# j04n-f/Encrypt-zkVM

Measured on AMD Instinct MI355X. Metric: STARK prove: trace-steps/sec at 2^20 steps; achieved HBM GB/s vs 8 TB/s peak, higher is better.
Workload: dtype f128

## Files before the change

encrypt-zkvm_amd/csrc/f128.hpp:

```cpp
#pragma once
#include <hip/hip_runtime.h>
#include <stdint.h>

#include "addsub_asm.hpp"

#define ZK_HD __host__ __device__ __forceinline__

struct fe {
    uint64_t lo, hi;
};

static constexpr uint64_t ZK_P_LO = 0xffffd30000000001ULL;
static constexpr uint64_t ZK_P_HI = 0xffffffffffffffffULL;
static constexpr uint64_t ZK_C = 0x2cffffffffffULL;

ZK_HD fe fe_make(uint64_t lo, uint64_t hi = 0) { return fe{lo, hi}; }
ZK_HD fe fe_zero() { return fe{0, 0}; }
ZK_HD fe fe_one() { return fe{1, 0}; }
ZK_HD bool fe_eq(fe a, fe b) { return a.lo == b.lo && a.hi == b.hi; }
ZK_HD bool fe_is_zero(fe a) { return (a.lo | a.hi) == 0; }

ZK_HD uint32_t lo32(uint64_t v) { return (uint32_t)v; }
ZK_HD uint32_t hi32(uint64_t v) { return (uint32_t)(v >> 32); }
ZK_HD uint64_t join32(uint32_t lo, uint32_t hi) { return (uint64_t)lo | ((uint64_t)hi << 32); }
// ... 553 lines not shown
#pragma unroll
    for (int k = 1; k < 8; k++) acc.w[k] = __builtin_addc(acc.w[k], r[k], c, &c);
    acc.w[8] += c;
}
ZK_HD fe acc288_reduce(const acc288 &acc) {
    const fe v = reduce_fold(acc.w[0], acc.w[1], acc.w[2], acc.w[3], acc.w[4], acc.w[5], acc.w[6], acc.w[7]);
    constexpr uint64_t C2_LO = (uint64_t)(((unsigned __int128)ZK_C * ZK_C) & ~0ULL);
    constexpr uint64_t C2_HI = (uint64_t)(((unsigned __int128)ZK_C * ZK_C) >> 64);
    const uint64_t t_lo = (uint64_t)lo32(C2_LO) * acc.w[8];
    const uint64_t t_mid = (uint64_t)hi32(C2_LO) * acc.w[8] + (t_lo >> 32);
    const uint64_t t_hi = C2_HI * acc.w[8] + (t_mid >> 32);
    const fe top = fe{(t_lo & 0xffffffffull) | (t_mid << 32), t_hi};
    return fe_add(v, top);
}

__device__ __forceinline__ fe fe_mul(fe a, fe b) { return fe_mul_asm(a, b); }
__host__ static inline fe fe_from_u128(unsigned __int128 v) { return fe{(uint64_t)v, (uint64_t)(v >> 64)}; }
__host__ static inline unsigned __int128 fe_to_u128(fe a) { return ((unsigned __int128)a.hi << 64) | a.lo; }
__host__ static inline fe fe_reduce_wide(unsigned __int128 lo, unsigned __int128 hi) {
    typedef unsigned __int128 u128;
    const u128 P = ((u128)ZK_P_HI << 64) | ZK_P_LO;
    const u128 t0 = (u128)(uint64_t)hi * ZK_C, t1 = (u128)(uint64_t)(hi >> 64) * ZK_C;
    const u128 s1 = lo + t0;
    const u128 s2 = s1 + (t1 << 64);
    const uint64_t top = (uint64_t)(t1 >> 64) + (uint64_t)(s1 < lo) + (uint64_t)(s2 < s1);
    u128 r = s2 + (u128)top * ZK_C;
    if (r < s2) r += ZK_C;
    if (r >= P) r -= P;
    return fe_from_u128(r);
}
// ... 111 lines not shown
```

encrypt-zkvm_amd/csrc/kernels.hip:

```cpp
#include <hip/hip_runtime.h>
#include <bitset>
#include <mutex>
#include <stdlib.h>
#include <string.h>

#include "blake3.hpp"
#include "fri_small.hpp"
#include "rescue_consts.hpp"
#include "zk_internal.hpp"

namespace zk {

#define ZK_LAUNCH_CHECK() (void)hipGetLastError()

static inline unsigned cdiv(size_t a, size_t b) { return (unsigned)((a + b - 1) / b); }

__device__ __forceinline__ fe ld_fe(const fe *p) { return *p; }
__device__ __forceinline__ void st_fe(fe *p, fe v) { *p = v; }

template <class T>
__device__ __forceinline__ T pow_split(const T *lo, const T *hi, size_t t) {
    return ChalOf<T>::mul(lo[t & 2047], hi[t >> 11]);
}

// ... 1316 lines not shown
                                468778791690ull, 208346129640ull, 22570830711ull, 573956280ull,
                                418414128120ull, 151093990710ull, 15496819560ull, 387420489ull};
    uint32_t pos[6] = {0x0u, 0x200u, 0xffa60000u, 0xffffffffu, 0xffffffffu, 0x1ffu}, neg[6] = {0, 0, 0, 0, 0, 0};
    acc192_madd(pos, y[0], A[4 * r + 0]);
    acc192_madd(neg, y[1], A[4 * r + 1]);
    acc192_madd(pos, y[2], A[4 * r + 2]);
    acc192_madd(neg, y[3], A[4 * r + 3]);
    uint32_t d[6], b;
    d[0] = __builtin_subc(pos[0], neg[0], 0u, &b);
#pragma unroll
    for (int k = 1; k < 6; k++) d[k] = __builtin_subc(pos[k], neg[k], b, &b);
    return reduce_fold(d[0], d[1], d[2], d[3], d[4], d[5], 0u, 0u);
}
static constexpr fe ZK_INV3_72 = fe{0x8092deb1ab776293ull, 0xf0185d00eca40a3bull};

struct EvalShared {
    fe ct[20], cb[22], ct2[20], cb2[22];
    fe ct3[4], nct[4], ct3b[4], nctb[4];
    fe u[4], ub[4];
    fe delta, bnd1, bnd1b;
};

#ifndef ZK_EVAL_LAZY
#define ZK_EVAL_LAZY 1
#endif
#ifndef ZK_EVAL_WAVES
#define ZK_EVAL_WAVES 4
#endif
#ifndef ZK_EVAL_WAVES_EXT
#define ZK_EVAL_WAVES_EXT 4
#endif
template <int KE, bool BND>
__global__ void __launch_bounds__(256, KE == 1 ? ZK_EVAL_WAVES : ZK_EVAL_WAVES_EXT) k_eval_constraints(const fe *lde, int log_n, EvalMap map, const fe *periodic,
                                                          const fe *divs, const AirConsts *K, const AirConsts *K2,
                                                          size_t plane, fe *comp) {
    __shared__ EvalShared S;
    __shared__ fe stash[4][256];
    const int tid = threadIdx.x;
    {
        const int t = threadIdx.x;
        if (t < 20) S.ct[t] = K->coeff_t[t];
        else if (t < 42) S.cb[t - 20] = K->coeff_b[t - 20];
        else if (t == 42) S.bnd1 = K->bnd1;
        else if (t == 43) S.bnd1b = KE == 2 ? K2->bnd1 : fe_zero();
        else if (t == 44) S.delta = K->delta;
        else if (t >= 80 && t < 84) {
            S.ct3[t - 80] = fe_mul(K->coeff_t[12 + t - 80], ZK_INV3_72);
            S.nct[t - 80] = fe_neg(K->coeff_t[12 + t - 80]);
        } else if (KE == 2 && t >= 84 && t < 88) {
            S.ct3b[t - 84] = fe_mul(K2->coeff_t[12 + t - 84], ZK_INV3_72);
            S.nctb[t - 84] = fe_neg(K2->coeff_t[12 + t - 84]);
        }
        else if (t >= 88 && t < 92) S.u[t - 88] = air_fold_mds(K->coeff_t + 12, t - 88);
        else if (KE == 2 && t >= 92 && t < 96) S.ub[t - 92] = air_fold_mds(K2->coeff_t + 12, t - 92);
        else if (KE == 2 && t >= 128 && t < 148) S.ct2[t - 128] = K2->coeff_t[t - 128];
        else if (KE == 2 && t >= 148 && t < 170) S.cb2[t - 148] = K2->coeff_b[t - 148];
        __syncthreads();
    }
    const int L = K->lwe_size;
    const size_t n = (size_t)1 << log_n;
    const size_t CE = n * map.nce;
    const size_t t_id = blockIdx.x * (size_t)blockDim.x + threadIdx.x;
    if (t_id >= CE) return;
    const size_t jl = t_id >> log_n, q = t_id & (n - 1), qn = (q + 1) & (n - 1);
    const size_t rc = map.ce0 + map.cestep * jl;
    const size_t i = rc + 8 * q;
    const size_t r = jl << map.lshift;
    const fe *cb = lde + r * n;
    const size_t cs = (size_t)map.lde_cosets * n;
#define CUR(c) cb[(size_t)(c)*cs + q]
#define NXT(c) cb[(size_t)(c)*cs + qn]
    const fe one = fe_one();
    fe t = fe_zero();
    fe t2 = fe_zero();
#define ZK_ACC(k, val)                                                    \
    do {                                                                  \
        const fe v_ = (val);                                              \
        t = fe_add(t, fe_mul(S.ct[k], v_));                               \
        if (KE == 2) {                                                    \
            t2 = fe_add(t2, fe_mul(S.ct2[k], v_));                        \
            asm volatile("" : "+v"(t2.lo), "+v"(t2.hi));                  \
        }                                                                 \
    } while (0)
    {
        constexpr bool LZ = KE == 1 && ZK_EVAL_LAZY;
        acc288 aS = acc288_zero();
#define ZK_ACCS(k, val)                                  \
    do {                                                 \
        if (LZ) acc288_madd(aS, S.ct[k], (val));    \
        else ZK_ACC(k, val);                             \
    } while (0)
#define ZK_SEQS() ZK_SEQ(cb, LZ ? aS.w[0] : (uint32_t)t.lo)
        const fe b0 = CUR(5), b1 = CUR(4), b2 = CUR(3), b3 = CUR(2), b4 = CUR(1);
        {
            fe opc = b0;
            opc = fe_add(fe_add(opc, opc), b1);
            opc = fe_add(fe_add(opc, opc), b2);
            opc = fe_add(fe_add(opc, opc), b3);
            opc = fe_add(fe_add(opc, opc), b4);
            stash[0][tid] = opc;
        }
        const fe nb0 = fe_sub(one, b0), nb2 = fe_sub(one, b2), nb3 = fe_sub(one, b3), nb4 = fe_sub(one, b4);
        const fe s0 = CUR(12), s1 = CUR(13);
        const fe s0n = NXT(12);
        ZK_ACCS(0, fe_sub(NXT(0), fe_add(CUR(0), one)));
        const fe b01 = fe_mul(b0, b1);
        ZK_ACCS(2, b01);
        const fe b0n1 = fe_sub(b0, b01);
        const fe n0_1 = fe_sub(b1, b01);
        const fe n01 = fe_sub(nb0, n0_1);
        {
            const fe is_noop = fe_mul(fe_mul(fe_mul(n01, nb2), nb3), nb4);
            ZK_ACCS(11, fe_mul(is_noop, fe_sub(s0n, s0)));
        }
        ZK_SEQS();
        const fe n0_1_b2 = fe_mul(n0_1, b2);
        const fe n0_1_n2 = fe_sub(n0_1, n0_1_b2);
        const fe Y = fe_mul(n0_1_n2, b3);
        fe is_add2, is_read2;
        {
            const fe X = fe_sub(n0_1_n2, Y);
            const fe e3 = fe_mul(S.ct[3], fe_sub(s0n, fe_add(s0, s1)));
            const fe e6 = fe_mul(S.ct[6], fe_sub(s0n, fe_mul(s0, s1)));
            const fe i36 = fe_add(e3, fe_mul(b4, fe_sub(e6, e3)));
            if (LZ) acc288_madd(aS, X, i36);
            else t = fe_add(t, fe_mul(X, i36));
            if (KE == 2) {
                const fe f3 = fe_mul(S.ct2[3], fe_sub(s0n, fe_add(s0, s1)));
                const fe f6 = fe_mul(S.ct2[6], fe_sub(s0n, fe_mul(s0, s1)));
                t2 = fe_add(t2, fe_mul(X, fe_add(f3, fe_mul(b4, fe_sub(f6, f3)))));
                asm volatile("" : "+v"(t2.lo), "+v"(t2.hi));
            }
        }
        ZK_SEQS();
        {
            is_add2 = fe_mul(Y, b4);
            const fe is_sadd = fe_sub(Y, is_add2);
            const fe is_smul = fe_mul(fe_mul(n0_1_b2, nb3), nb4);
            fe sum_sn = fe_zero(), sum_s1 = fe_zero(), sum_hi = fe_zero();
            for (int k = 0; k < L; k++) {
                sum_sn = fe_add(sum_sn, NXT(12 + k));
                sum_s1 = fe_add(sum_s1, CUR(13 + k));
            }
            for (int k = 1; k < L; k++) sum_hi = fe_add(sum_hi, CUR(12 + L + k));
            const fe base = fe_sub(sum_sn, sum_s1);
            const fe acc7 = fe_sub(sum_sn, fe_mul(sum_s1, s0));
            const fe acc4 = fe_sub(base, fe_mul(S.delta, s0));
            const fe acc5 = fe_sub(base, fe_add(s0, sum_hi));
            ZK_ACCS(4, fe_mul(is_sadd, acc4));
            ZK_ACCS(5, fe_mul(is_add2, acc5));
            ZK_ACCS(7, fe_mul(is_smul, acc7));
        }
        ZK_SEQS();
        {
            const fe p0 = fe_mul(b0n1, nb2);
            const fe p0b3 = fe_mul(p0, b3);
            const fe p0n3 = fe_sub(p0, p0b3);
            stash[1][tid] = fe_mul(s0n, fe_mul(p0n3, nb4));
            is_read2 = fe_mul(p0b3, nb4);
            const fe zd1 = fe_mul(p0n3, fe_sub(NXT(13), s0));
            const fe i89 = fe_add(S.ct[8], fe_mul(b4, fe_sub(S.ct[9], S.ct[8])));
            if (LZ) acc288_madd(aS, zd1, i89);
            else t = fe_add(t, fe_mul(zd1, i89));
            if (KE == 2) {
                t2 = fe_add(t2, fe_mul(zd1, fe_add(S.ct2[8], fe_mul(b4, fe_sub(S.ct2[9], S.ct2[8])))));
                asm volatile("" : "+v"(t2.lo), "+v"(t2.hi));
            }
            ZK_ACCS(10, fe_mul(is_read2, fe_sub(NXT(17), s0)));
        }
        {
            fe v = fe_add(fe_sub(fe_sub(NXT(11), CUR(11)), b0), b1);
            fe d = fe_sub(is_add2, is_read2);
            d = fe_add(d, d);
            d = fe_add(d, d);
            ZK_ACCS(1, fe_add(v, d));
        }
        if (LZ) t = fe_add(t, acc288_reduce(aS));
#undef ZK_ACCS
#undef ZK_SEQS
    }
    ZK_SEQ(cb, t.lo);
    {
        const fe opc = stash[0][tid], push_term = stash[1][tid];
        const fe *per = periodic + (i & 127) * 9;
        acc288 aR = acc288_zero(), aR2 = acc288_zero();
        {
            const fe pv = K->pv[i & 127];
            aR.w[0] = lo32(pv.lo), aR.w[1] = hi32(pv.lo), aR.w[2] = lo32(pv.hi), aR.w[3] = hi32(pv.hi);
            acc288_madd(aR, S.nct[0], opc);
            acc288_madd(aR, S.nct[1], push_term);
            if (KE == 2) {
                const fe pvb = K2->pv[i & 127];
                aR2.w[0] = lo32(pvb.lo), aR2.w[1] = hi32(pvb.lo), aR2.w[2] = lo32(pvb.hi), aR2.w[3] = hi32(pvb.hi);
                acc288_madd(aR2, S.nctb[0], opc);
                acc288_madd(aR2, S.nctb[1], push_term);
            }
        }
#pragma unroll
        for (int k = 0; k < 4; k++) {
            const fe c = CUR(7 + k);
            if (k < 2) stash[2 + k][tid] = c;
            const fe x = cube(c);
            acc288_madd(aR, S.u[k], x);
            if (KE == 2) acc288_madd(aR2, S.ub[k], x);
        }
        ZK_SEQ(cb, aR.w[0]);
        const fe h0 = CUR(6);
        const fe fh = fe_mul(per[0], h0);
        const fe nfh = fe_sub(h0, fh);
        fe y[4];
#pragma unroll
        for (int k = 0; k < 4; k++) y[k] = fe_sub(NXT(7 + k), per[5 + k]);
        fe sR = fe_zero(), sR2 = fe_zero();
        {
#pragma unroll
            for (int r2 = 0; r2 < 4; r2++) {
                const fe v3 = cube(adj_row(r2, y));
                acc288_madd(aR, S.ct3[r2], v3);
                if (KE == 2) acc288_madd(aR2, S.ct3b[r2], v3);
            }
            sR = acc288_reduce(aR);
            if (KE == 2) sR2 = acc288_reduce(aR2);
        }
        t = fe_add(t, fe_mul(sR, fh));
        if (KE == 2) t2 = fe_add(t2, fe_mul(sR2, fh));
        ZK_SEQ(cb, t.lo);
        {
            const fe c7 = stash[2][tid], c8 = stash[3][tid];
            const fe d16 = fe_sub(NXT(7), c7), d17 = fe_sub(NXT(8), c8), n9 = NXT(9), n10 = NXT(10);
            acc288 aC = acc288_zero();
            acc288_madd(aC, S.ct[16], d16);
            acc288_madd(aC, S.ct[17], d17);
            acc288_madd(aC, S.ct[18], n9);
            acc288_madd(aC, S.ct[19], n10);
            t = fe_add(t, fe_mul(acc288_reduce(aC), nfh));
            if (KE == 2) {
                acc288 aD = acc288_zero();
                acc288_madd(aD, S.ct2[16], d16);
                acc288_madd(aD, S.ct2[17], d17);
                acc288_madd(aD, S.ct2[18], n9);
                acc288_madd(aD, S.ct2[19], n10);
                t2 = fe_add(t2, fe_mul(acc288_reduce(aD), nfh));
            }
        }
    }
    ZK_SEQ(cb, t.lo);
    const size_t P = map.dplane ? map.dplane : CE;
    const fe dT = divs[t_id];
    if constexpr (!BND) {
        comp[t_id] = fe_mul(t, dT);
        if (KE == 2) comp[plane + t_id] = fe_mul(t2, dT);
    } else {
        const fe d0 = divs[P + t_id], d1 = divs[2 * P + t_id];
        acc288 a0 = acc288_zero(), a1 = acc288_zero();
        acc288_madd(a0, S.cb[0], CUR(0));
        acc288_madd(a0, S.cb[1], CUR(7));
        acc288_madd(a0, S.cb[2], CUR(8));
        acc288_madd(a0, S.cb[3], CUR(11));
        acc288_madd(a1, S.cb[12], CUR(7));
        acc288_madd(a1, S.cb[13], CUR(8));
#pragma unroll
        for (int k = 0; k < 8; k++) {
            fe c = CUR(12 + k);
            acc288_madd(a0, S.cb[4 + k], c);
            acc288_madd(a1, S.cb[14 + k], c);
        }
        const fe bs0 = acc288_reduce(a0), bs1 = fe_sub(acc288_reduce(a1), S.bnd1);
        acc288 aR = acc288_zero();
        acc288_madd(aR, t, dT);
        acc288_madd(aR, bs0, d0);
        acc288_madd(aR, bs1, d1);
        const fe res = acc288_reduce(aR);
        comp[t_id] = res;
        if (KE == 2) {
            ZK_SEQ(cb, res.lo);
            acc288 c0 = acc288_zero(), c1 = acc288_zero();
            acc288_madd(c0, S.cb2[0], CUR(0));
            acc288_madd(c0, S.cb2[1], CUR(7));
            acc288_madd(c0, S.cb2[2], CUR(8));
            acc288_madd(c0, S.cb2[3], CUR(11));
            acc288_madd(c1, S.cb2[12], CUR(7));
            acc288_madd(c1, S.cb2[13], CUR(8));
#pragma unroll
            for (int k = 0; k < 8; k++) {
                fe c = CUR(12 + k);
                acc288_madd(c0, S.cb2[4 + k], c);
                acc288_madd(c1, S.cb2[14 + k], c);
            }
            const fe bs0b = acc288_reduce(c0), bs1b = fe_sub(acc288_reduce(c1), S.bnd1b);
            acc288 aR2 = acc288_zero();
            acc288_madd(aR2, t2, dT);
            acc288_madd(aR2, bs0b, d0);
            acc288_madd(aR2, bs1b, d1);
            comp[plane + t_id] = acc288_reduce(aR2);
        }
    }
#undef ZK_ACC
#undef CUR
#undef NXT
}

static std::mutex g_consts_mu;
static std::bitset<256> g_consts_done;
hipError_t upload_rescue_consts(hipStream_t st) {
    int dev = 0;
    hipError_t e = hipGetDevice(&dev);
    if (e != hipSuccess) return e;
    if (dev < 0 || dev >= 256) return hipErrorInvalidDevice;
    std::lock_guard<std::mutex> lk(g_consts_mu);
    if (g_consts_done.test((size_t)dev)) return hipSuccess;
    fe m[16];
// ... 178 lines not shown
            atomicMin(&rep->t_first[tid], mn);
        }
    } else if (tid == 20) {
        atomicAdd(&rep->failing_steps, (unsigned long long)sh_steps[0] + sh_steps[1] + sh_steps[2] + sh_steps[3]);
    }
}

hipError_t validate_trace(hipStream_t st, const fe *trace, size_t n, const fe *per_tab, fe delta, int lwe_size,
                          ValReport *rep) {
    const size_t steps = n - 2;
    ZK_PROF(st, "validate_trace", 448.0 * n, hipLaunchKernelGGL(k_validate_trace, dim3(cdiv(steps, 256)), dim3(256), 0, st,
                                                                trace, n, per_tab, delta, lwe_size, rep));
    return hipGetLastError();
}

__global__ void __launch_bounds__(256) k_comp_cross(CrossMap m, const fe *wi_lo, const fe *wi_hi,
                                                    const fe *i3_lo, const fe *i3_hi, fe scale, fe w8inv,
                                                    fe inv3n, int ncols, fe *polys, unsigned *nonzero) {
    for (size_t kl = blockIdx.x * (size_t)blockDim.x + threadIdx.x; kl < m.kcount; kl += (size_t)gridDim.x * blockDim.x) {
        const size_t k1 = m.k0 + kl;
        fe w = pow_split(wi_lo, wi_hi, k1);
        fe d[8];
        fe wr = fe_one();
#pragma unroll
        for (int r = 0; r < 8; r++) {
            if (r == 7 && m.derive7) {
                acc288 a7 = acc288_zero();
#pragma unroll
                for (int j = 0; j < 7; j++) acc288_madd(a7, m.k7[j], d[j]);
                d[7] = acc288_reduce(a7);
                break;
            }
            fe v = m.c[r][kl];
            d[r] = r ? fe_mul(v, wr) : v;
            wr = fe_mul(wr, w);
        }
        fe w2 = fe_mul(w8inv, w8inv), w3 = fe_mul(w2, w8inv);
        fe e0 = d[0], e1 = d[4], e2 = d[2], e3 = d[6], e4 = d[1], e5 = d[5], e6 = d[3], e7 = d[7];
        fe t0 = fe_add(e0, e1), t1 = fe_sub(e0, e1), t2 = fe_add(e2, e3), t3 = fe_sub(e2, e3);
        fe t4 = fe_add(e4, e5), t5 = fe_sub(e4, e5), t6 = fe_add(e6, e7), t7 = fe_sub(e6, e7);
        t3 = fe_mul(t3, w2);
        t7 = fe_mul(t7, w2);
        fe u0 = fe_add(t0, t2), u2 = fe_sub(t0, t2), u1 = fe_add(t1, t3), u3 = fe_sub(t1, t3);
        fe u4 = fe_add(t4, t6), u6 = fe_sub(t4, t6), u5 = fe_add(t5, t7), u7 = fe_sub(t5, t7);
        u5 = fe_mul(u5, w8inv);
        u6 = fe_mul(u6, w2);
        u7 = fe_mul(u7, w3);
        fe bk[8] = {fe_add(u0, u4), fe_add(u1, u5), fe_add(u2, u6), fe_add(u3, u7),
                    fe_sub(u0, u4), fe_sub(u1, u5), fe_sub(u2, u6), fe_sub(u3, u7)};
        fe s = fe_mul(scale, pow_split(i3_lo, i3_hi, k1));
        unsigned nz = 0;
#pragma unroll
        for (int k2 = 0; k2 < 8; k2++) {
            fe a = fe_mul(bk[k2], s);
            if (k2 < ncols) polys[(size_t)k2 * m.pstride + kl] = a;
            else nz |= !fe_is_zero(a);
            s = fe_mul(s, inv3n);
        }
        if (nz) atomicOr(nonzero, 1u);
    }
}

void comp_cross_mapped(hipStream_t st, const CrossMap &m, const NttTables &T8n, const PowTable &inv3, fe scale,
                       fe w8inv, fe inv3n, int ncols, fe *polys, unsigned *nonzero_flag) {
    unsigned blocks = cdiv(m.kcount, 256);
    if (blocks > 65536) blocks = 65536;
    ZK_PROF(st, "comp_cross", (128.0 + 16.0 * ncols) * m.kcount, hipLaunchKernelGGL(k_comp_cross, dim3(blocks), dim3(256), 0, st, m, T8n.inv_lo,
                                                 T8n.inv_hi, inv3.lo, inv3.hi, scale, w8inv, inv3n, ncols, polys,
                                                 nonzero_flag));
}

constexpr int OOD_GROUP = 7;

template <int KX>
__global__ void k_ood_tables(typename Chal<KX>::T z, typename Chal<KX>::T zg, uint64_t chunk, int nw,
                             typename Chal<KX>::T *tab) {
    typedef typename Chal<KX>::T T;
    const int t = blockIdx.x * blockDim.x + threadIdx.x;
    if (t >= 128 + 2 * nw) return;
    T x;
    uint64_t e;
    if (t < 128) {
        x = t < 64 ? z : zg;
// ... 663 lines not shown
        if (op == 14) fe_mul_wsv2(x, ws[t], a[mir], ws[mir], o[0], o[1]);
        else fe_mul_w2_2(x, w2[t], a[mir], w2[mir], o[0], o[1]);
        r = o[t & 1];
        break;
    }
    case 16: r = ws_fold(lo32(x.lo), hi32(x.lo), lo32(x.hi), hi32(x.hi), lo32(y.lo), hi32(y.lo) & 7u); break;
    case 17: {
        const fe x2 = a[mir], y2 = b[mir];
        uint32_t A[4] = {lo32(x.lo), hi32(x.lo), lo32(x.hi), hi32(x.hi)};
        uint32_t B[4] = {lo32(x2.lo), hi32(x2.lo), lo32(x2.hi), hi32(x2.hi)};
        fe o[2];
        ws_fold2(A, lo32(y.lo), hi32(y.lo) & 7u, B, lo32(y2.lo), hi32(y2.lo) & 7u, o[0], o[1]);
        r = o[t & 1];
        break;
    }
    case 0: r = fe_add(x, y); break;
    case 1: r = fe_sub(x, y); break;
    case 2: r = fe_mul(x, y); break;
    case 3: r = fe_inv(x); break;
    case 5: r = fe_add_lazy(x, y); break;
    case 6: r = fe_canon(x); break;
    case 7: r = fe_mul_w2(x, fe_w2{y, fe_mul(y, fe{0, 1})}); break;
    case 8:
    case 9:
    case 10: {
        const fe x2 = a[count - 1 - t], y2 = b[count - 1 - t];
        fe o[4];
        if (op == 8) addsub2_v<0>(x, y, x2, y2, o[0], o[1], o[2], o[3]);
        else if (op == 9) addsub2_v<1>(x, y, x2, y2, o[0], o[1], o[2], o[3]);
        else addsub2_v<2>(x, y, x2, y2, o[0], o[1], o[2], o[3]);
// ... 25 lines not shown
```

encrypt-zkvm_amd/csrc/prover.hip:

```cpp
#include <hip/hip_runtime.h>
#include <stdio.h>
#include <string.h>

#include <algorithm>
#include <chrono>
#include <cstdlib>
#include <map>
#include <memory>
#include <new>
#include <string>
#include <vector>

#include "host_pool.hpp"
#include "prover_internal.hpp"
#include "rescue_consts.hpp"

namespace zk {
thread_local std::string g_err;
struct HostTimer {
    bool on = getenv("ZK_HOST_TIMING") != nullptr;
    std::chrono::steady_clock::time_point t = std::chrono::steady_clock::now();
    std::string log;
    void start() { t = std::chrono::steady_clock::now(); }
    void lap(const char *what) { stop(what), start(); }
// ... 734 lines not shown
    e.push_back(fe_make(((uint64_t)opt->field_extension << 16) | ((uint64_t)opt->fri_folding << 8) | opt->fri_rem_max_deg));
    e.push_back(fe_make(opt->grinding));
    e.push_back(fe_make(opt->blowup));
    e.push_back(fe_make(opt->num_queries));
    for (int i = 0; i < 2; i++) e.push_back(fe_from_bytes(pub->program_hash[i]));
    for (int i = 0; i < 16; i++) e.push_back(fe_from_bytes(pub->stack_outputs[i]));
    Coin coin;
    coin.init(e);
    return coin;
}

static void set_coeff_derived(AirConsts &K, const fe *per) {
    K.bnd1 = fe_zero();
    for (int k = 12; k < NUM_ASSERTS; k++) K.bnd1 = fe_add(K.bnd1, fe_mul(K.coeff_b[k], K.assert_val[k]));
    air_fold_periodic(K.coeff_t + 12, per, K.pv);
}

static const fe *air_static_consts(const zk_pub_inputs *pub, size_t n, AirConsts &K) {
    const int log_n = ilog2(n);
    const int first_cols[12] = {0, 7, 8, 11, 12, 13, 14, 15, 16, 17, 18, 19};
    int k = 0;
    for (int i = 0; i < 12; i++, k++) {
        K.assert_col[k] = first_cols[i];
        K.assert_grp[k] = 0;
        K.assert_val[k] = fe_zero();
    }
    for (int i = 0; i < 2; i++, k++) {
        K.assert_col[k] = 7 + i;
        K.assert_grp[k] = 1;
        K.assert_val[k] = fe_from_bytes(pub->program_hash[i]);
// ... 1164 lines not shown
    for (size_t i = 0; i < count; i++) acc288_madd(acc, fe_from_bytes(a + 16 * i), fe_from_bytes(b + 16 * i));
    fe_to_bytes(acc288_reduce(acc), out);
}

extern "C" void zk_diag_mul_limbs_host(const uint8_t *a, const uint8_t *b, uint8_t *out, size_t count) {
    for (size_t i = 0; i < count; i++) fe_to_bytes(fe_mul_limbs(fe_from_bytes(a + 16 * i), fe_from_bytes(b + 16 * i)), out + 16 * i);
}
extern "C" void zk_diag_air_fold_host(const uint8_t *ct, size_t n, uint8_t *u_out, uint8_t *pv_out) {
    fe c[4], pv[128];
    for (int r = 0; r < 4; r++) c[r] = fe_from_bytes(ct + 16 * r);
    for (int k = 0; k < 4; k++) fe_to_bytes(air_fold_mds(c, k), u_out + 16 * k);
    const std::vector<fe> per = periodic_table(n);
    air_fold_periodic(c, per.data(), pv);
    for (int j = 0; j < 128; j++) fe_to_bytes(pv[j], pv_out + 16 * j);
}
extern "C" void zk_diag_blake3_host(const uint8_t *in, size_t len, uint8_t out[32]) { b3::hash_bytes(in, len, out); }

static UploadPlanIn diag_upload_plan_in(const uint32_t *in, size_t n) {
    UploadPlanIn q;
    q.have = in[0], q.sparse = in[1], q.nw8 = in[2], q.nw32 = in[3], q.clk_off = in[4], q.fixed_off = in[5];
    q.snap = in[6], q.snap_mask = in[7], q.hint_ok = in[8], q.no_virtual = in[9], q.lat_sched = in[10], q.detect = in[11];
    q.sparse_on = in[12] & 1u, q.narrow_on = in[12] & 2u, q.clock_on = in[12] & 4u, q.fixed_on = in[12] & 8u;
    q.fixed_fuse_on = in[12] & 16u, q.virtual_on = in[12] & 32u, q.coeff_src_on = in[12] & 64u;
    q.n = n;
    return q;
}
extern "C" int zk_diag_upload_plan_coeff_src(const uint32_t *in, size_t n) {
    return upload_plan(diag_upload_plan_in(in, n)).coeff_src ? 1 : 0;
}
extern "C" int zk_diag_upload_plan(const uint32_t *in, size_t n, uint32_t *masks, int32_t *counts, int32_t *cols,
// ... 39 lines not shown
    if (!idx || !out || (G != 2 && G != 4 && G != 8) || M < 8 * (uint64_t)G || (M & (M - 1)))
        ZK_FAIL(ZK_ERR_INVALID_ARG, "zk_diag_shard_locate: G = 2, 4 or 8, M a power of two >= 8 G");
    TreeGeom T;
    T.shape(M, G);
    for (size_t i = 0; i < count; i++) {
        if (is_node ? (idx[i] < 1 || idx[i] >= M) : idx[i] >= M)
            ZK_FAIL(ZK_ERR_INVALID_ARG, "zk_diag_shard_locate: leaf index below M, heap node index in 1 .. M - 1");
        const TreeGeom::Loc L = T.locate(is_node, idx[i]);
        out[3 * i] = L.owner, out[3 * i + 1] = L.which, out[3 * i + 2] = (int64_t)L.off;
    }
    return ZK_OK;
}

extern "C" int zk_diag_field_op(int device, int op, const uint8_t *a, const uint8_t *b, uint8_t *out, size_t count) {
    if (!a || !b || !out || count == 0) ZK_FAIL(ZK_ERR_INVALID_ARG, "null argument");
    if (op < 0 || op > 17 || count > ((size_t)1 << 30) || (op == 13 && count % 64 != 0))
        ZK_FAIL(ZK_ERR_INVALID_ARG, "zk_diag_field_op: unknown op, or a count the op does not take");
    ZK_CHECK_HIP(hipSetDevice(device));
    std::vector<fe_ws> ws;
    std::vector<fe_w2> w2;
    if (op >= 11 && op <= 14) {
        ws.resize(count);
        for (size_t i = 0; i < count; i++) ws[i] = make_fe_ws(fe_from_bytes(b + 16 * i));
    } else if (op == 15) {
        w2.resize(count);
        for (size_t i = 0; i < count; i++) w2[i] = make_fe_w2(fe_from_bytes(b + 16 * i));
    }
    fe *d = nullptr;
    void *tab = nullptr;
    const size_t tab_bytes = ws.size() * sizeof(fe_ws) + w2.size() * sizeof(fe_w2);
    ZK_CHECK_HIP(hipMalloc(&d, 3 * count * sizeof(fe)));
    hipError_t e = tab_bytes ? hipMalloc(&tab, tab_bytes) : hipSuccess;
    if (e == hipSuccess) e = hipMemcpy(d, a, count * 16, hipMemcpyHostToDevice);
    if (e == hipSuccess) e = hipMemcpy(d + count, b, count * 16, hipMemcpyHostToDevice);
    if (e == hipSuccess && tab_bytes)
        e = hipMemcpy(tab, ws.empty() ? (const void *)w2.data() : (const void *)ws.data(), tab_bytes, hipMemcpyHostToDevice);
// ... 473 lines not shown
```

encrypt-zkvm_amd/csrc/zk_internal.hpp:

```cpp
#pragma once
#include <hip/hip_runtime.h>
#include <stddef.h>
#include <stdint.h>

#include <string>
#include <vector>

#include "chal.hpp"
#include "f128.hpp"

namespace zk {

struct KernelProfiler {
    bool on = false;
    struct Rec {
        const char *name;
        hipEvent_t a, b;
        double bytes;
        double muls, addsubs;
    };
    std::vector<Rec> recs;
    std::vector<hipEvent_t> pool;
    size_t used = 0;
    hipEvent_t get() {
// ... 149 lines not shown
                 fe *out);

struct AirConsts {
    fe coeff_t[20];
    fe coeff_b[22];
    int assert_col[22];
    int assert_grp[22];
    fe assert_val[22];
    fe inv_zn[8];
    fe xr[8];
    fe g_last2, g_last1;
    fe delta;
    fe bnd1;
    int lwe_size;
    fe pv[128];
};
ZK_HD uint32_t mds_abs(int i) {
    constexpr uint32_t M[16] = {729, 1080, 390, 40, 29160, 42471, 14520, 1210,
                                882090, 1277640, 429429, 33880, 24698520, 35708310, 11935560, 925771};
    return M[i];
}
ZK_HD fe air_fold_mds(const fe *ct, int k) {
    acc160 a = acc160_zero();
    for (int r = 0; r < 4; r++) acc160_madd(a, ct[r], mds_abs(4 * r + k));
    const fe s = acc160_reduce(a);
    return (k & 1) ? fe_neg(s) : s;
}
inline void air_fold_periodic(const fe *ct, const fe *per, fe pv[128]) {
    const fe nct[4] = {fe_neg(ct[0]), fe_neg(ct[1]), fe_neg(ct[2]), fe_neg(ct[3])};
    for (int j = 0; j < 128; j++) {
        fe s = fe_zero();
// ... 124 lines not shown
```

Baseline: 119.8 million.

## Precompute uniform-constant multiplier tables on host and use 192-bit accumulators in eval

Constraint-evaluation constants are precomputed on the host into fe_ws tables stored in AirConsts, and the kernel multiplies by them with fe_mul_uniform / acc192_madd_uniform loaded through scalar registers. This removes the shared-memory staging block and its __syncthreads. The narrower acc192 accumulator replaces acc288 wherever the term count allows. A few products are also reordered (n34 and p0 hoisted, the stash reused for v), and k_comp_cross gets precomputed twiddle tables. It adds host-side setup and a larger AirConsts struct, and relies on the uniform-multiply path being cheaper than generic fe_mul.

```diff
diff --git a/encrypt-zkvm_amd/csrc/f128.hpp b/encrypt-zkvm_amd/csrc/f128.hpp
--- a/encrypt-zkvm_amd/csrc/f128.hpp
+++ b/encrypt-zkvm_amd/csrc/f128.hpp
@@ -591,6 +591,39 @@
     return fe_add(v, top);
 }
 
+constexpr int ACC192_MAX_TERMS = 1 << 15;
+struct acc192 {
+    uint32_t w[6];
+};
+__device__ __forceinline__ acc192 acc192_zero() { return acc192{{0, 0, 0, 0, 0, 0}}; }
+__device__ __forceinline__ acc192 acc192_from(fe v) { return acc192{{lo32(v.lo), hi32(v.lo), lo32(v.hi), hi32(v.hi), 0, 0}}; }
+__device__ __forceinline__ void acc192_madd_uniform(acc192 &acc, fe x, const fe_ws &W) {
+    uint32_t r[4], s4, s5, c;
+    asm volatile("" : "+v"(x.lo), "+v"(x.hi) : "v"(acc.w[0]));
+    ws_columns_s(x, W, r, s4, s5);
+    acc.w[0] = __builtin_addc(acc.w[0], r[0], 0u, &c);
+#pragma unroll
+    for (int k = 1; k < 4; k++) acc.w[k] = __builtin_addc(acc.w[k], r[k], c, &c);
+    acc.w[4] = __builtin_addc(acc.w[4], s4, c, &c);
+    acc.w[5] += s5 + c;
+}
+__device__ __forceinline__ fe acc192_reduce(const acc192 &acc) {
+    return ws_fold(acc.w[0], acc.w[1], acc.w[2], acc.w[3], acc.w[4], acc.w[5]);
+}
+__device__ __forceinline__ void acc288_madd_uniform(acc288 &acc, fe x, const fe_ws &W) {
+    uint32_t r[4], s4, s5, c;
+    asm volatile("" : "+v"(x.lo), "+v"(x.hi) : "v"(acc.w[0]));
+    ws_columns_s(x, W, r, s4, s5);
+    acc.w[0] = __builtin_addc(acc.w[0], r[0], 0u, &c);
+#pragma unroll
+    for (int k = 1; k < 4; k++) acc.w[k] = __builtin_addc(acc.w[k], r[k], c, &c);
+    acc.w[4] = __builtin_addc(acc.w[4], s4, c, &c);
+    acc.w[5] = __builtin_addc(acc.w[5], s5, c, &c);
+    acc.w[6] = __builtin_addc(acc.w[6], 0u, c, &c);
+    acc.w[7] = __builtin_addc(acc.w[7], 0u, c, &c);
+    acc.w[8] += c;
+}
+
 __device__ __forceinline__ fe fe_mul(fe a, fe b) { return fe_mul_asm(a, b); }
 __host__ static inline fe fe_from_u128(unsigned __int128 v) { return fe{(uint64_t)v, (uint64_t)(v >> 64)}; }
 __host__ static inline unsigned __int128 fe_to_u128(fe a) { return ((unsigned __int128)a.hi << 64) | a.lo; }
diff --git a/encrypt-zkvm_amd/csrc/kernels.hip b/encrypt-zkvm_amd/csrc/kernels.hip
--- a/encrypt-zkvm_amd/csrc/kernels.hip
+++ b/encrypt-zkvm_amd/csrc/kernels.hip
@@ -1354,12 +1354,15 @@
 }
 static constexpr fe ZK_INV3_72 = fe{0x8092deb1ab776293ull, 0xf0185d00eca40a3bull};
 
-struct EvalShared {
-    fe ct[20], cb[22], ct2[20], cb2[22];
-    fe ct3[4], nct[4], ct3b[4], nctb[4];
-    fe u[4], ub[4];
-    fe delta, bnd1, bnd1b;
-};
+void air_build_ws(AirConsts &K) {
+    for (int k = 0; k < 20; k++)
+        K.ws[EW_CT + k] = make_fe_ws(k >= 12 && k < 16 ? fe_mul(K.coeff_t[k], ZK_INV3_72) : K.coeff_t[k]);
+    for (int r = 0; r < 2; r++) K.ws[EW_NCT + r] = make_fe_ws(fe_neg(K.coeff_t[12 + r]));
+    for (int k = 0; k < 4; k++) K.ws[EW_U + k] = make_fe_ws(air_fold_mds(K.coeff_t + 12, k));
+    K.ws[EW_D89] = make_fe_ws(fe_sub(K.coeff_t[9], K.coeff_t[8]));
+    K.ws[EW_DELTA] = make_fe_ws(K.delta);
+    for (int k = 0; k < 22; k++) K.ws[EW_CB + k] = make_fe_ws(K.coeff_b[k]);
+}
 
 #ifndef ZK_EVAL_LAZY
 #define ZK_EVAL_LAZY 1
@@ -1372,32 +1375,15 @@
 #endif
 template <int KE, bool BND>
 __global__ void __launch_bounds__(256, KE == 1 ? ZK_EVAL_WAVES : ZK_EVAL_WAVES_EXT) k_eval_constraints(const fe *lde, int log_n, EvalMap map, const fe *periodic,
-                                                          const fe *divs, const AirConsts *K, const AirConsts *K2,
-                                                          size_t plane, fe *comp) {
-    __shared__ EvalShared S;
+                                                          const fe *divs, const AirConsts *__restrict__ K,
+                                                          const AirConsts *__restrict__ K2, size_t plane,
+                                                          fe *comp) {
     __shared__ fe stash[4][256];
     const int tid = threadIdx.x;
-    {
-        const int t = threadIdx.x;
-        if (t < 20) S.ct[t] = K->coeff_t[t];
-        else if (t < 42) S.cb[t - 20] = K->coeff_b[t - 20];
-        else if (t == 42) S.bnd1 = K->bnd1;
-        else if (t == 43) S.bnd1b = KE == 2 ? K2->bnd1 : fe_zero();
-        else if (t == 44) S.delta = K->delta;
-        else if (t >= 80 && t < 84) {
-            S.ct3[t - 80] = fe_mul(K->coeff_t[12 + t - 80], ZK_INV3_72);
-            S.nct[t - 80] = fe_neg(K->coeff_t[12 + t - 80]);
-        } else if (KE == 2 && t >= 84 && t < 88) {
-            S.ct3b[t - 84] = fe_mul(K2->coeff_t[12 + t - 84], ZK_INV3_72);
-            S.nctb[t - 84] = fe_neg(K2->coeff_t[12 + t - 84]);
-        }
-        else if (t >= 88 && t < 92) S.u[t - 88] = air_fold_mds(K->coeff_t + 12, t - 88);
-        else if (KE == 2 && t >= 92 && t < 96) S.ub[t - 92] = air_fold_mds(K2->coeff_t + 12, t - 92);
-        else if (KE == 2 && t >= 128 && t < 148) S.ct2[t - 128] = K2->coeff_t[t - 128];
-        else if (KE == 2 && t >= 148 && t < 170) S.cb2[t - 148] = K2->coeff_b[t - 148];
-        __syncthreads();
-    }
     const int L = K->lwe_size;
+    int wo = 0;
+#define ZK_WA(idx) load_fe_ws(K->ws, wo + (idx))
+#define ZK_WB(idx) load_fe_ws(K2->ws, wo + (idx))
     const size_t n = (size_t)1 << log_n;
     const size_t CE = n * map.nce;
     const size_t t_id = blockIdx.x * (size_t)blockDim.x + threadIdx.x;
@@ -1413,24 +1399,29 @@
     const fe one = fe_one();
     fe t = fe_zero();
     fe t2 = fe_zero();
-#define ZK_ACC(k, val)                                                    \
-    do {                                                                  \
-        const fe v_ = (val);                                              \
-        t = fe_add(t, fe_mul(S.ct[k], v_));                               \
-        if (KE == 2) {                                                    \
-            t2 = fe_add(t2, fe_mul(S.ct2[k], v_));                        \
-            asm volatile("" : "+v"(t2.lo), "+v"(t2.hi));                  \
-        }                                                                 \
+#define ZK_SEQK(dep)                            \
+    do {                                        \
+        ZK_SEQ(cb, dep);                        \
+        asm volatile("" : "+s"(wo) : "v"(dep)); \
+    } while (0)
+#define ZK_ACC(k, val)                                                        \
+    do {                                                                      \
+        const fe v_ = (val);                                                  \
+        t = fe_add(t, fe_mul_uniform(v_, ZK_WA(EW_CT + (k))));                \
+        if (KE == 2) {                                                        \
+            t2 = fe_add(t2, fe_mul_uniform(v_, ZK_WB(EW_CT + (k))));          \
+            asm volatile("" : "+v"(t2.lo), "+v"(t2.hi));                      \
+        }                                                                     \
     } while (0)
     {
         constexpr bool LZ = KE == 1 && ZK_EVAL_LAZY;
         acc288 aS = acc288_zero();
-#define ZK_ACCS(k, val)                                  \
-    do {                                                 \
-        if (LZ) acc288_madd(aS, S.ct[k], (val));    \
-        else ZK_ACC(k, val);                             \
+#define ZK_ACCS(k, val)                                                 \
+    do {                                                                \
+        if (LZ) acc288_madd_uniform(aS, (val), ZK_WA(EW_CT + (k)));     \
+        else ZK_ACC(k, val);                                            \
     } while (0)
-#define ZK_SEQS() ZK_SEQ(cb, LZ ? aS.w[0] : (uint32_t)t.lo)
+#define ZK_SEQS() ZK_SEQK(LZ ? aS.w[0] : (uint32_t)t.lo)
         const fe b0 = CUR(5), b1 = CUR(4), b2 = CUR(3), b3 = CUR(2), b4 = CUR(1);
         {
             fe opc = b0;
@@ -1445,29 +1436,34 @@
         const fe s0n = NXT(12);
         ZK_ACCS(0, fe_sub(NXT(0), fe_add(CUR(0), one)));
         const fe b01 = fe_mul(b0, b1);
+        stash[2][tid] = fe_add(fe_sub(NXT(11), CUR(11)), fe_sub(b1, b0));
         ZK_ACCS(2, b01);
         const fe b0n1 = fe_sub(b0, b01);
         const fe n0_1 = fe_sub(b1, b01);
         const fe n01 = fe_sub(nb0, n0_1);
+        const fe n34 = fe_mul(nb3, nb4);
         {
-            const fe is_noop = fe_mul(fe_mul(fe_mul(n01, nb2), nb3), nb4);
+            const fe is_noop = fe_mul(fe_mul(n01, nb2), n34);
             ZK_ACCS(11, fe_mul(is_noop, fe_sub(s0n, s0)));
         }
         ZK_SEQS();
+        const fe p0 = fe_mul(b0n1, nb2);
         const fe n0_1_b2 = fe_mul(n0_1, b2);
         const fe n0_1_n2 = fe_sub(n0_1, n0_1_b2);
+        const fe is_smul = fe_mul(n0_1_b2, n34);
         const fe Y = fe_mul(n0_1_n2, b3);
         fe is_add2, is_read2;
         {
             const fe X = fe_sub(n0_1_n2, Y);
-            const fe e3 = fe_mul(S.ct[3], fe_sub(s0n, fe_add(s0, s1)));
-            const fe e6 = fe_mul(S.ct[6], fe_sub(s0n, fe_mul(s0, s1)));
+            const fe d3 = fe_sub(s0n, fe_add(s0, s1)), d6 = fe_sub(s0n, fe_mul(s0, s1));
+            const fe e3 = fe_mul_uniform(d3, ZK_WA(EW_CT + 3));
+            const fe e6 = fe_mul_uniform(d6, ZK_WA(EW_CT + 6));
             const fe i36 = fe_add(e3, fe_mul(b4, fe_sub(e6, e3)));
             if (LZ) acc288_madd(aS, X, i36);
             else t = fe_add(t, fe_mul(X, i36));
             if (KE == 2) {
-                const fe f3 = fe_mul(S.ct2[3], fe_sub(s0n, fe_add(s0, s1)));
-                const fe f6 = fe_mul(S.ct2[6], fe_sub(s0n, fe_mul(s0, s1)));
+                const fe f3 = fe_mul_uniform(d3, ZK_WB(EW_CT + 3));
+                const fe f6 = fe_mul_uniform(d6, ZK_WB(EW_CT + 6));
                 t2 = fe_add(t2, fe_mul(X, fe_add(f3, fe_mul(b4, fe_sub(f6, f3)))));
                 asm volatile("" : "+v"(t2.lo), "+v"(t2.hi));
             }
@@ -1476,7 +1472,6 @@
         {
             is_add2 = fe_mul(Y, b4);
             const fe is_sadd = fe_sub(Y, is_add2);
-            const fe is_smul = fe_mul(fe_mul(n0_1_b2, nb3), nb4);
             fe sum_sn = fe_zero(), sum_s1 = fe_zero(), sum_hi = fe_zero();
             for (int k = 0; k < L; k++) {
                 sum_sn = fe_add(sum_sn, NXT(12 + k));
@@ -1485,7 +1480,7 @@
             for (int k = 1; k < L; k++) sum_hi = fe_add(sum_hi, CUR(12 + L + k));
             const fe base = fe_sub(sum_sn, sum_s1);
             const fe acc7 = fe_sub(sum_sn, fe_mul(sum_s1, s0));
-            const fe acc4 = fe_sub(base, fe_mul(S.delta, s0));
+            const fe acc4 = fe_sub(base, fe_mul_uniform(s0, ZK_WA(EW_DELTA)));
             const fe acc5 = fe_sub(base, fe_add(s0, sum_hi));
             ZK_ACCS(4, fe_mul(is_sadd, acc4));
             ZK_ACCS(5, fe_mul(is_add2, acc5));
@@ -1493,23 +1488,22 @@
         }
         ZK_SEQS();
         {
-            const fe p0 = fe_mul(b0n1, nb2);
             const fe p0b3 = fe_mul(p0, b3);
             const fe p0n3 = fe_sub(p0, p0b3);
             stash[1][tid] = fe_mul(s0n, fe_mul(p0n3, nb4));
             is_read2 = fe_mul(p0b3, nb4);
             const fe zd1 = fe_mul(p0n3, fe_sub(NXT(13), s0));
-            const fe i89 = fe_add(S.ct[8], fe_mul(b4, fe_sub(S.ct[9], S.ct[8])));
+            const fe i89 = fe_add(K->coeff_t[8], fe_mul_uniform(b4, ZK_WA(EW_D89)));
             if (LZ) acc288_madd(aS, zd1, i89);
             else t = fe_add(t, fe_mul(zd1, i89));
             if (KE == 2) {
-                t2 = fe_add(t2, fe_mul(zd1, fe_add(S.ct2[8], fe_mul(b4, fe_sub(S.ct2[9], S.ct2[8])))));
+                t2 = fe_add(t2, fe_mul(zd1, fe_add(K2->coeff_t[8], fe_mul_uniform(b4, ZK_WB(EW_D89)))));
                 asm volatile("" : "+v"(t2.lo), "+v"(t2.hi));
             }
             ZK_ACCS(10, fe_mul(is_read2, fe_sub(NXT(17), s0)));
         }
         {
-            fe v = fe_add(fe_sub(fe_sub(NXT(11), CUR(11)), b0), b1);
+            const fe v = stash[2][tid];
             fe d = fe_sub(is_add2, is_read2);
             d = fe_add(d, d);
             d = fe_add(d, d);
@@ -1519,32 +1513,27 @@
 #undef ZK_ACCS
 #undef ZK_SEQS
     }
-    ZK_SEQ(cb, t.lo);
+    ZK_SEQK(t.lo);
     {
         const fe opc = stash[0][tid], push_term = stash[1][tid];
         const fe *per = periodic + (i & 127) * 9;
-        acc288 aR = acc288_zero(), aR2 = acc288_zero();
-        {
-            const fe pv = K->pv[i & 127];
-            aR.w[0] = lo32(pv.lo), aR.w[1] = hi32(pv.lo), aR.w[2] = lo32(pv.hi), aR.w[3] = hi32(pv.hi);
-            acc288_madd(aR, S.nct[0], opc);
-            acc288_madd(aR, S.nct[1], push_term);
-            if (KE == 2) {
-                const fe pvb = K2->pv[i & 127];
-                aR2.w[0] = lo32(pvb.lo), aR2.w[1] = hi32(pvb.lo), aR2.w[2] = lo32(pvb.hi), aR2.w[3] = hi32(pvb.hi);
-                acc288_madd(aR2, S.nctb[0], opc);
-                acc288_madd(aR2, S.nctb[1], push_term);
-            }
+        acc192 aR = acc192_from(K->pv[i & 127]), aR2 = acc192_zero();
+        acc192_madd_uniform(aR, opc, ZK_WA(EW_NCT + 0));
+        acc192_madd_uniform(aR, push_term, ZK_WA(EW_NCT + 1));
+        if (KE == 2) {
+            aR2 = acc192_from(K2->pv[i & 127]);
+            acc192_madd_uniform(aR2, opc, ZK_WB(EW_NCT + 0));
+            acc192_madd_uniform(aR2, push_term, ZK_WB(EW_NCT + 1));
         }
 #pragma unroll
         for (int k = 0; k < 4; k++) {
             const fe c = CUR(7 + k);
             if (k < 2) stash[2 + k][tid] = c;
             const fe x = cube(c);
-            acc288_madd(aR, S.u[k], x);
-            if (KE == 2) acc288_madd(aR2, S.ub[k], x);
-        }
-        ZK_SEQ(cb, aR.w[0]);
+            acc192_madd_uniform(aR, x, ZK_WA(EW_U + k));
+            if (KE == 2) acc192_madd_uniform(aR2, x, ZK_WB(EW_U + k));
+        }
+        ZK_SEQK(aR.w[0]);
         const fe h0 = CUR(6);
         const fe fh = fe_mul(per[0], h0);
         const fe nfh = fe_sub(h0, fh);
@@ -1556,35 +1545,35 @@
 #pragma unroll
             for (int r2 = 0; r2 < 4; r2++) {
                 const fe v3 = cube(adj_row(r2, y));
-                acc288_madd(aR, S.ct3[r2], v3);
-                if (KE == 2) acc288_madd(aR2, S.ct3b[r2], v3);
+                acc192_madd_uniform(aR, v3, ZK_WA(EW_CT + 12 + r2));
+                if (KE == 2) acc192_madd_uniform(aR2, v3, ZK_WB(EW_CT + 12 + r2));
             }
-            sR = acc288_reduce(aR);
-            if (KE == 2) sR2 = acc288_reduce(aR2);
+            sR = acc192_reduce(aR);
+            if (KE == 2) sR2 = acc192_reduce(aR2);
         }
         t = fe_add(t, fe_mul(sR, fh));
         if (KE == 2) t2 = fe_add(t2, fe_mul(sR2, fh));
-        ZK_SEQ(cb, t.lo);
+        ZK_SEQK(t.lo);
         {
             const fe c7 = stash[2][tid], c8 = stash[3][tid];
             const fe d16 = fe_sub(NXT(7), c7), d17 = fe_sub(NXT(8), c8), n9 = NXT(9), n10 = NXT(10);
-            acc288 aC = acc288_zero();
-            acc288_madd(aC, S.ct[16], d16);
-            acc288_madd(aC, S.ct[17], d17);
-            acc288_madd(aC, S.ct[18], n9);
-            acc288_madd(aC, S.ct[19], n10);
-            t = fe_add(t, fe_mul(acc288_reduce(aC), nfh));
+            acc192 aC = acc192_zero();
+            acc192_madd_uniform(aC, d16, ZK_WA(EW_CT + 16));
+            acc192_madd_uniform(aC, d17, ZK_WA(EW_CT + 17));
+            acc192_madd_uniform(aC, n9, ZK_WA(EW_CT + 18));
+            acc192_madd_uniform(aC, n10, ZK_WA(EW_CT + 19));
+            t = fe_add(t, fe_mul(acc192_reduce(aC), nfh));
             if (KE == 2) {
-                acc288 aD = acc288_zero();
-                acc288_madd(aD, S.ct2[16], d16);
-                acc288_madd(aD, S.ct2[17], d17);
-                acc288_madd(aD, S.ct2[18], n9);
-                acc288_madd(aD, S.ct2[19], n10);
-                t2 = fe_add(t2, fe_mul(acc288_reduce(aD), nfh));
+                acc192 aD = acc192_zero();
+                acc192_madd_uniform(aD, d16, ZK_WB(EW_CT + 16));
+                acc192_madd_uniform(aD, d17, ZK_WB(EW_CT + 17));
+                acc192_madd_uniform(aD, n9, ZK_WB(EW_CT + 18));
+                acc192_madd_uniform(aD, n10, ZK_WB(EW_CT + 19));
+                t2 = fe_add(t2, fe_mul(acc192_reduce(aD), nfh));
             }
         }
     }
-    ZK_SEQ(cb, t.lo);
+    ZK_SEQK(t.lo);
     const size_t P = map.dplane ? map.dplane : CE;
     const fe dT = divs[t_id];
     if constexpr (!BND) {
@@ -1592,20 +1581,24 @@
         if (KE == 2) comp[plane + t_id] = fe_mul(t2, dT);
     } else {
         const fe d0 = divs[P + t_id], d1 = divs[2 * P + t_id];
-        acc288 a0 = acc288_zero(), a1 = acc288_zero();
-        acc288_madd(a0, S.cb[0], CUR(0));
-        acc288_madd(a0, S.cb[1], CUR(7));
-        acc288_madd(a0, S.cb[2], CUR(8));
-        acc288_madd(a0, S.cb[3], CUR(11));
-        acc288_madd(a1, S.cb[12], CUR(7));
-        acc288_madd(a1, S.cb[13], CUR(8));
-#pragma unroll
-        for (int k = 0; k < 8; k++) {
-            fe c = CUR(12 + k);
-            acc288_madd(a0, S.cb[4 + k], c);
-            acc288_madd(a1, S.cb[14 + k], c);
-        }
-        const fe bs0 = acc288_reduce(a0), bs1 = fe_sub(acc288_reduce(a1), S.bnd1);
+        auto bnd_sums = [&](const AirConsts *__restrict__ Kp, fe &bs0, fe &bs1) {
+            acc192 a0 = acc192_zero(), a1 = acc192_zero();
+            acc192_madd_uniform(a0, CUR(0), load_fe_ws(Kp->ws, wo + EW_CB + 0));
+            acc192_madd_uniform(a0, CUR(7), load_fe_ws(Kp->ws, wo + EW_CB + 1));
+            acc192_madd_uniform(a0, CUR(8), load_fe_ws(Kp->ws, wo + EW_CB + 2));
+            acc192_madd_uniform(a0, CUR(11), load_fe_ws(Kp->ws, wo + EW_CB + 3));
+            acc192_madd_uniform(a1, CUR(7), load_fe_ws(Kp->ws, wo + EW_CB + 12));
+            acc192_madd_uniform(a1, CUR(8), load_fe_ws(Kp->ws, wo + EW_CB + 13));
+#pragma unroll
+            for (int k = 0; k < 8; k++) {
+                const fe c = CUR(12 + k);
+                acc192_madd_uniform(a0, c, load_fe_ws(Kp->ws, wo + EW_CB + 4 + k));
+                acc192_madd_uniform(a1, c, load_fe_ws(Kp->ws, wo + EW_CB + 14 + k));
+            }
+            bs0 = acc192_reduce(a0), bs1 = fe_sub(acc192_reduce(a1), Kp->bnd1);
+        };
+        fe bs0, bs1;
+        bnd_sums(K, bs0, bs1);
         acc288 aR = acc288_zero();
         acc288_madd(aR, t, dT);
         acc288_madd(aR, bs0, d0);
@@ -1613,21 +1606,9 @@
         const fe res = acc288_reduce(aR);
         comp[t_id] = res;
         if (KE == 2) {
-            ZK_SEQ(cb, res.lo);
-            acc288 c0 = acc288_zero(), c1 = acc288_zero();
-            acc288_madd(c0, S.cb2[0], CUR(0));
-            acc288_madd(c0, S.cb2[1], CUR(7));
-            acc288_madd(c0, S.cb2[2], CUR(8));
-            acc288_madd(c0, S.cb2[3], CUR(11));
-            acc288_madd(c1, S.cb2[12], CUR(7));
-            acc288_madd(c1, S.cb2[13], CUR(8));
-#pragma unroll
-            for (int k = 0; k < 8; k++) {
-                fe c = CUR(12 + k);
-                acc288_madd(c0, S.cb2[4 + k], c);
-                acc288_madd(c1, S.cb2[14 + k], c);
-            }
-            const fe bs0b = acc288_reduce(c0), bs1b = fe_sub(acc288_reduce(c1), S.bnd1b);
+            ZK_SEQK(res.lo);
+            fe bs0b, bs1b;
+            bnd_sums(K2, bs0b, bs1b);
             acc288 aR2 = acc288_zero();
             acc288_madd(aR2, t2, dT);
             acc288_madd(aR2, bs0b, d0);
@@ -1635,6 +1616,9 @@
             comp[plane + t_id] = acc288_reduce(aR2);
         }
     }
+#undef ZK_SEQK
+#undef ZK_WA
+#undef ZK_WB
 #undef ZK_ACC
 #undef CUR
 #undef NXT
@@ -1843,9 +1827,12 @@
     return hipGetLastError();
 }
 
+struct CrossWs {
+    fe_ws w1, w2, w3, inv3n, k7[7];
+};
 __global__ void __launch_bounds__(256) k_comp_cross(CrossMap m, const fe *wi_lo, const fe *wi_hi,
-                                                    const fe *i3_lo, const fe *i3_hi, fe scale, fe w8inv,
-                                                    fe inv3n, int ncols, fe *polys, unsigned *nonzero) {
+                                                    const fe *i3_lo, const fe *i3_hi, fe scale, CrossWs cw,
+                                                    int ncols, fe *polys, unsigned *nonzero) {
     for (size_t kl = blockIdx.x * (size_t)blockDim.x + threadIdx.x; kl < m.kcount; kl += (size_t)gridDim.x * blockDim.x) {
         const size_t k1 = m.k0 + kl;
         fe w = pow_split(wi_lo, wi_hi, k1);
@@ -1854,27 +1841,26 @@
 #pragma unroll
         for (int r = 0; r < 8; r++) {
             if (r == 7 && m.derive7) {
-                acc288 a7 = acc288_zero();
-#pragma unroll
-                for (int j = 0; j < 7; j++) acc288_madd(a7, m.k7[j], d[j]);
-                d[7] = acc288_reduce(a7);
+                acc192 a7 = acc192_zero();
+#pragma unroll
+                for (int j = 0; j < 7; j++) acc192_madd_uniform(a7, d[j], cw.k7[j]);
+                d[7] = acc192_reduce(a7);
                 break;
             }
             fe v = m.c[r][kl];
             d[r] = r ? fe_mul(v, wr) : v;
             wr = fe_mul(wr, w);
         }
-        fe w2 = fe_mul(w8inv, w8inv), w3 = fe_mul(w2, w8inv);
         fe e0 = d[0], e1 = d[4], e2 = d[2], e3 = d[6], e4 = d[1], e5 = d[5], e6 = d[3], e7 = d[7];
         fe t0 = fe_add(e0, e1), t1 = fe_sub(e0, e1), t2 = fe_add(e2, e3), t3 = fe_sub(e2, e3);
         fe t4 = fe_add(e4, e5), t5 = fe_sub(e4, e5), t6 = fe_add(e6, e7), t7 = fe_sub(e6, e7);
-        t3 = fe_mul(t3, w2);
-        t7 = fe_mul(t7, w2);
+        t3 = fe_mul_uniform(t3, cw.w2);
+        t7 = fe_mul_uniform(t7, cw.w2);
         fe u0 = fe_add(t0, t2), u2 = fe_sub(t0, t2), u1 = fe_add(t1, t3), u3 = fe_sub(t1, t3);
         fe u4 = fe_add(t4, t6), u6 = fe_sub(t4, t6), u5 = fe_add(t5, t7), u7 = fe_sub(t5, t7);
-        u5 = fe_mul(u5, w8inv);
-        u6 = fe_mul(u6, w2);
-        u7 = fe_mul(u7, w3);
+        u5 = fe_mul_uniform(u5, cw.w1);
+        u6 = fe_mul_uniform(u6, cw.w2);
+        u7 = fe_mul_uniform(u7, cw.w3);
         fe bk[8] = {fe_add(u0, u4), fe_add(u1, u5), fe_add(u2, u6), fe_add(u3, u7),
                     fe_sub(u0, u4), fe_sub(u1, u5), fe_sub(u2, u6), fe_sub(u3, u7)};
         fe s = fe_mul(scale, pow_split(i3_lo, i3_hi, k1));
@@ -1884,7 +1870,7 @@
             fe a = fe_mul(bk[k2], s);
             if (k2 < ncols) polys[(size_t)k2 * m.pstride + kl] = a;
             else nz |= !fe_is_zero(a);
-            s = fe_mul(s, inv3n);
+            s = fe_mul_uniform(s, cw.inv3n);
         }
         if (nz) atomicOr(nonzero, 1u);
     }
@@ -1894,8 +1880,13 @@
                        fe w8inv, fe inv3n, int ncols, fe *polys, unsigned *nonzero_flag) {
     unsigned blocks = cdiv(m.kcount, 256);
     if (blocks > 65536) blocks = 65536;
+    CrossWs cw;
+    const fe w2 = fe_mul(w8inv, w8inv);
+    cw.w1 = make_fe_ws(w8inv), cw.w2 = make_fe_ws(w2), cw.w3 = make_fe_ws(fe_mul(w2, w8inv));
+    cw.inv3n = make_fe_ws(inv3n);
+    for (int j = 0; j < 7; j++) cw.k7[j] = make_fe_ws(m.k7[j]);
     ZK_PROF(st, "comp_cross", (128.0 + 16.0 * ncols) * m.kcount, hipLaunchKernelGGL(k_comp_cross, dim3(blocks), dim3(256), 0, st, m, T8n.inv_lo,
-                                                 T8n.inv_hi, inv3.lo, inv3.hi, scale, w8inv, inv3n, ncols, polys,
+                                                 T8n.inv_hi, inv3.lo, inv3.hi, scale, cw, ncols, polys,
                                                  nonzero_flag));
 }
 
@@ -2589,6 +2580,29 @@
         r = o[t & 1];
         break;
     }
+    case 18:
+    case 19: {
+        const fe_ws Wc = load_fe_ws(ws, (int)w0);
+        acc192 s = acc192_from(x);
+        acc288 s2 = acc288_zero();
+        if (op == 19) acc288_madd(s2, x, y);
+#pragma unroll 1
+        for (int j = 0; j < 16; j++) {
+            const fe v = a[(t + j) % count];
+            if (op == 18) acc192_madd_uniform(s, v, Wc);
+            else acc288_madd_uniform(s2, v, Wc);
+        }
+        r = op == 18 ? acc192_reduce(s) : acc288_reduce(s2);
+        break;
+    }
+    case 20: {
+        const fe_ws Wc = load_fe_ws(ws, (int)w0);
+        acc192 s = acc192_from(x);
+#pragma unroll 1
+        for (int j = 0; j < ACC192_MAX_TERMS; j++) acc192_madd_uniform(s, x, Wc);
+        r = acc192_reduce(s);
+        break;
+    }
     case 0: r = fe_add(x, y); break;
     case 1: r = fe_sub(x, y); break;
     case 2: r = fe_mul(x, y); break;
diff --git a/encrypt-zkvm_amd/csrc/prover.hip b/encrypt-zkvm_amd/csrc/prover.hip
--- a/encrypt-zkvm_amd/csrc/prover.hip
+++ b/encrypt-zkvm_amd/csrc/prover.hip
@@ -772,6 +772,7 @@
     K.bnd1 = fe_zero();
     for (int k = 12; k < NUM_ASSERTS; k++) K.bnd1 = fe_add(K.bnd1, fe_mul(K.coeff_b[k], K.assert_val[k]));
     air_fold_periodic(K.coeff_t + 12, per, K.pv);
+    air_build_ws(K);
 }
 
 static const fe *air_static_consts(const zk_pub_inputs *pub, size_t n, AirConsts &K) {
@@ -1966,6 +1967,15 @@
     air_fold_periodic(c, per.data(), pv);
     for (int j = 0; j < 128; j++) fe_to_bytes(pv[j], pv_out + 16 * j);
 }
+extern "C" void zk_diag_air_ws_host(const uint8_t *ct, const uint8_t *cb, const uint8_t *delta, uint8_t *out) {
+    AirConsts K;
+    memset(&K, 0, sizeof K);
+    for (int k = 0; k < NUM_TCONS; k++) K.coeff_t[k] = fe_from_bytes(ct + 16 * k);
+    for (int k = 0; k < NUM_ASSERTS; k++) K.coeff_b[k] = fe_from_bytes(cb + 16 * k);
+    K.delta = fe_from_bytes(delta);
+    air_build_ws(K);
+    memcpy(out, K.ws, sizeof K.ws);
+}
 extern "C" void zk_diag_blake3_host(const uint8_t *in, size_t len, uint8_t out[32]) { b3::hash_bytes(in, len, out); }
 
 static UploadPlanIn diag_upload_plan_in(const uint32_t *in, size_t n) {
@@ -2035,12 +2045,12 @@
 
 extern "C" int zk_diag_field_op(int device, int op, const uint8_t *a, const uint8_t *b, uint8_t *out, size_t count) {
     if (!a || !b || !out || count == 0) ZK_FAIL(ZK_ERR_INVALID_ARG, "null argument");
-    if (op < 0 || op > 17 || count > ((size_t)1 << 30) || (op == 13 && count % 64 != 0))
+    if (op < 0 || op > 20 || count > ((size_t)1 << 30) || (op == 13 && count % 64 != 0))
         ZK_FAIL(ZK_ERR_INVALID_ARG, "zk_diag_field_op: unknown op, or a count the op does not take");
     ZK_CHECK_HIP(hipSetDevice(device));
     std::vector<fe_ws> ws;
     std::vector<fe_w2> w2;
-    if (op >= 11 && op <= 14) {
+    if ((op >= 11 && op <= 14) || op >= 18) {
         ws.resize(count);
         for (size_t i = 0; i < count; i++) ws[i] = make_fe_ws(fe_from_bytes(b + 16 * i));
     } else if (op == 15) {
diff --git a/encrypt-zkvm_amd/csrc/zk_internal.hpp b/encrypt-zkvm_amd/csrc/zk_internal.hpp
--- a/encrypt-zkvm_amd/csrc/zk_internal.hpp
+++ b/encrypt-zkvm_amd/csrc/zk_internal.hpp
@@ -187,7 +187,11 @@
     fe bnd1;
     int lwe_size;
     fe pv[128];
-};
+    fe_ws ws[50];
+};
+enum EvalWs { EW_CT = 0, EW_NCT = 20, EW_U = 22, EW_D89 = 26, EW_DELTA = 27, EW_CB = 28, EW_COUNT = 50 };
+static_assert(EW_COUNT == sizeof(AirConsts::ws) / sizeof(fe_ws), "AirConsts::ws holds one W set per EvalWs index");
+void air_build_ws(AirConsts &K);
 ZK_HD uint32_t mds_abs(int i) {
     constexpr uint32_t M[16] = {729, 1080, 390, 40, 29160, 42471, 14520, 1210,
                                 882090, 1277640, 429429, 33880, 24698520, 35708310, 11935560, 925771};
```

Result: faster. 122.1 million, median of 6 (+1.9%).
